# yynil/RWKV_LM_EXT

Measured on AMD Instinct MI355X. Metric: WKV6 fwd+bwd tokens/sec/GPU (B=8,T=4096,C=2048) + %HBM roofline, higher is better.
Workload: dtype bf16

## Files before the change

### rwkv_lm_ext_amd/csrc/wkv6_chunk_bwd12k.hip

```cpp
#include <type_traits>
#include "wkv6_chunk.h"

namespace wkv6 {

namespace {

using namespace chunk;

enum { R_RH = 0, R_RL, R_GY, R_R, R_K, NR_ARR };
enum { K_KH = 0, K_KL, K_V, NK_ARR };
constexpr int FRS = 72 * 4;
constexpr int ROFF_FR = NR_ARR * ARR;
constexpr int ROFF_LW = ROFF_FR + BLK * FRS;
constexpr int ROFF_E8 = ROFF_LW + BLK * FRS;
constexpr int ROFF_COEF = ROFF_E8 + 256;
constexpr int ROFF_VG = ROFF_COEF + 128;
constexpr int RBLK_BYTES = ROFF_VG + 128;
constexpr int KOFF_E16 = NK_ARR * ARR;
constexpr int KOFF_E16M8 = KOFF_E16 + 256;
constexpr int KBLK_BYTES = KOFF_E16M8 + 256;
constexpr int STG = 32, SBLK = STG / BLK;
constexpr int RBUF_BYTES = SBLK * RBLK_BYTES;
constexpr int KBUF_BYTES = SBLK * KBLK_BYTES;
constexpr int KRING = 3;
constexpr int KP_OFF = 2 * RBUF_BYTES;
constexpr int CKT = CKPT_TOK;
constexpr int XT_OFF = KP_OFF + KRING * KBUF_BYTES;
constexpr int XS_OFF = XT_OFF + 4 * 1024;
constexpr int XFLAG_OFF = 128;
constexpr int GRS = 144;
constexpr int GOP_OFF = XS_OFF + 2 * 1024;
constexpr int TAG_DA = 0, TAG_SC = 4, TAG_GA = 8, TAG_GB = 12, TAG_GC = 16, TAG_GD = 20, N_TAGS = 24;
constexpr int BWD12K_LDS = GOP_OFF + 2 * HEAD * GRS;
static_assert(BWD12K_LDS <= 160 * 1024, "LDS budget");

#define WKV6_DPP_ACC4(x, ctrl) asm("s_nop 1\n\t" \
    "v_add_f32_dpp %0, %0, %0 " ctrl " row_mask:0xf bank_mask:0xf\n\t" "v_add_f32_dpp %1, %1, %1 " ctrl " row_mask:0xf bank_mask:0xf\n\t" \
    "v_add_f32_dpp %2, %2, %2 " ctrl " row_mask:0xf bank_mask:0xf\n\t" "v_add_f32_dpp %3, %3, %3 " ctrl " row_mask:0xf bank_mask:0xf" \
    : "+v"(x[0]), "+v"(x[1]), "+v"(x[2]), "+v"(x[3]))

enum : unsigned {
    BWD_W_RAW = 1u << 0,
    BWD_SPLIT = 1u << 1,
    BWD_AFF = 1u << 2,
    BWD_CLK = 1u << 3,
    BWD_CHAIN = 1u << 4,
    BWD_VARLEN = 1u << 5,
};
constexpr unsigned bit(bool on, unsigned b) { return on ? b : 0u; }
struct BwdChain {
    int b, ntok;
    int ko, ro;
    bool chained_in;
    bool nx_chain;
    unsigned nx_bh;
    int nx_b, nx_ntok;
    bool nx_rev, nx_use_u;
    const float* nx_ckpt;
};
struct BwdCarry {
    uint2 pr[2], pk[2], pw[2];
    float4 pe[2];
    uint2 ck_[2];
    float cfr[2][4], clw[2][4], cc8[4];
    uint2 cvp[2];
    f4v CK[4];
};
template <unsigned MODE, int GEN = 0, int ROLE = 0>
__device__ __forceinline__ void chunk_bwd12k_body(const ScanArgs& a, const unsigned slot, BwdCarry& cy, const unsigned sslot = 0, const BwdChain& ch = BwdChain{})
{
    constexpr bool W_RAW = (MODE & BWD_W_RAW) != 0;
    constexpr bool SPLIT = (MODE & BWD_SPLIT) != 0;
    constexpr bool AFF = (MODE & BWD_AFF) != 0;
    constexpr bool CLK = (MODE & BWD_CLK) != 0;
    constexpr bool CHAIN = (MODE & BWD_CHAIN) != 0;
    constexpr bool VARLEN = (MODE & BWD_VARLEN) != 0;
    [[maybe_unused]] const bool chained_in = CHAIN && ch.chained_in, nx_chain = CHAIN && ch.nx_chain;
    [[maybe_unused]] const int ko = CHAIN ? ch.ko : 0, ro = CHAIN ? ch.ro : 0;
    extern __shared__ __attribute__((aligned(16))) char smem[];
    int tid_ = threadIdx.x;
    if constexpr (CHAIN) asm volatile("" : "+v"(tid_));
    const int tid = tid_, lane = tid & 63;
    const SplitForms spf = split_forms(lane);
    const int hwid = __builtin_amdgcn_readfirstlane(tid >> 6);
    const int part = SPLIT ? (int)(slot & 1) : 0;
    const int bh = SPLIT ? (int)(slot >> 1) : (int)slot;
    const int wid = SPLIT ? (hwid < 4 ? hwid + 4 * part : hwid + 4) : hwid;
    const bool rowrole = ROLE ? ROLE == 1 : wid < 4, producer = ROLE ? ROLE == 3 : wid >= 8;
    const int wv = wid & 3;
    const int pb = wid & 1, half = (wid >> 1) & 1;
    const int b = CHAIN ? ch.b : (a.order ? a.order[bh / a.H] : bh / a.H), h = bh % a.H;
    const long base = VARLEN ? (long)a.tok_off[b] * a.C + (long)h * HEAD : (long)b * a.T * a.C + (long)h * HEAD;
    const bf16_t* const gr_ = reinterpret_cast<const bf16_t*>(a.r) + base;
    const bf16_t* const gk_ = reinterpret_cast<const bf16_t*>(a.k) + base;
    const bf16_t* const gv_ = reinterpret_cast<const bf16_t*>(a.v) + base;
    const bf16_t* const ggy = reinterpret_cast<const bf16_t*>(a.gy) + base;
    bf16_t* const ogr = reinterpret_cast<bf16_t*>(a.gr) + base;
    bf16_t* const ogk = reinterpret_cast<bf16_t*>(a.gk) + base;
    bf16_t* const ogv = reinterpret_cast<bf16_t*>(a.gv) + base;
    bf16_t* const ogw = reinterpret_cast<bf16_t*>(a.gw) + base;
    int ntok = a.T;
    if constexpr (CHAIN) ntok = ch.ntok;
    else if (a.lens) ntok = min(max(a.lens[b], 0), a.T);
    const TokAddr<AFF> tok(a, b, ntok);
    const int C_ = a.C;
    const unsigned nbytes = ntok > 0 ? (unsigned)(ntok - 1) * a.C * 2u + 128u : 0u;
    const rsrc_t rs_gr = make_rsrc(ogr, nbytes), rs_gk = make_rsrc(ogk, nbytes), rs_gv = make_rsrc(ogv, nbytes), rs_gw = make_rsrc(ogw, nbytes);
    const long sbase = (GEN && a.side_compact) ? (long)sslot * a.T * HEAD : base;
    const unsigned sstr = (GEN && a.side_compact) ? (unsigned)HEAD : (unsigned)a.C;
    const unsigned nbytes4 = ntok > 0 ? (unsigned)(ntok - 1) * sstr * 4u + 256u : 0u;
    const rsrc_t rs_side[4] = {make_rsrc(GEN && a.g_f32[0] ? a.g_f32[0] + sbase : nullptr, GEN && a.g_f32[0] ? nbytes4 : 0u),
                               make_rsrc(GEN && a.g_f32[1] ? a.g_f32[1] + sbase : nullptr, GEN && a.g_f32[1] ? nbytes4 : 0u),
                               make_rsrc(GEN && a.g_f32[2] ? a.g_f32[2] + sbase : nullptr, GEN && a.g_f32[2] ? nbytes4 : 0u),
                               make_rsrc(GEN && a.g_f32[3] ? a.g_f32[3] + sbase : nullptr, GEN && a.g_f32[3] ? nbytes4 : 0u)};
    const int lp_side = tok.lane(lane & 15, 16 * wv + 4 * (lane >> 4), (int)sstr);
    const int lp_put = tok.lane((((lane >> 4) & 1) ? 0 : BLK) + (lane & 15), 16 * wv + 8 * (lane >> 5), C_);
    auto fetch_old = [&](int which, const rsrc_t& rs, int pu, unsigned bit, float (&old)[4]) {
        if constexpr (GEN == 2) {
            const unsigned idx = tok.off(pu, lane & 15, 16 * wv + 4 * (lane >> 4), (int)sstr, bit, lp_side);
            const float4 t = buf_load16f(rs_side[which], idx * 4u);
            old[0] = t.x; old[1] = t.y; old[2] = t.z; old[3] = t.w;
        }
    };
#ifdef WKV6_STAMP
    unsigned long long stamp_acc[6] = {0, 0, 0, 0, 0, 0}, ts0 = 0, ts1 = 0, ts2 = 0, ts3 = 0, ts4 = 0, ts5 = 0;
    unsigned long long tp0 = 0, tp1 = 0;
    unsigned long long poll_acc[8] = {0, 0, 0, 0, 0, 0, 0, 0};
#define WKV6_ACCP(idx, t1, t0) do { stamp_acc[5] += (t1) - (t0); poll_acc[(idx) >> 2] += (t1) - (t0); } while (0)
#else
#define WKV6_ACCP(idx, t1, t0) do { } while (0)
#endif
    const int x_ = lane & 15, g_ = lane >> 4;
    typedef unsigned v2u_t __attribute__((ext_vector_type(2)));
    typedef unsigned v4u_t __attribute__((ext_vector_type(4)));
    typedef volatile v4u_t __attribute__((address_space(3))) lds_vv4u;
    [[maybe_unused]] uint2 held_st[4] = {};
    auto put = [&](int which, const rsrc_t& rs, int stg, int blk, unsigned bit, uint2 v) {
        if constexpr (GEN == 1) return;
        if (blk == SBLK - 1) { held_st[which] = v; return; }
        const auto sx = __builtin_amdgcn_permlane16_swap(held_st[which].x, v.x, false, false);
        const auto sy = __builtin_amdgcn_permlane16_swap(held_st[which].y, v.y, false, false);
        buf_store16(rs, tok.off(stg * STG, ((g_ & 1) ? 0 : BLK) + x_, 16 * wv + 8 * (g_ >> 1), C_, bit, lp_put) * 2u,
                    make_uint4(sx[0], sy[0], sx[1], sy[1]));
    };
    auto emit = [&](int which, int stg, int blk, unsigned bit, float (&o)[4], const float (&old)[4]) -> uint2 {
        if constexpr (GEN == 1) {
            const unsigned idx = tok.off(stg * STG + blk * BLK, x_, 16 * wv + 4 * g_, (int)sstr, bit, lp_side);
            buf_store16f(rs_side[which], idx * 4u, o);
            return make_uint2(0u, 0u);
        }
        if constexpr (GEN == 2) {
#pragma unroll
            for (int q = 0; q < 4; ++q) o[q] += old[q];
        }
        return make_uint2(pack_bf2(o[0], o[1]), pack_bf2(o[2], o[3]));
    };

#ifdef WKV6_DEBUGBUF
    unsigned long long clk0 = 0, rtc0 = 0, clk1 = 0, rtc1 = 0;
    WKV6_CLK(clk0, rtc0);
#endif
    if constexpr (CLK) { if (hwid == 0) clock_stamp(a, slot, 0); }
    const int ngrp = (ntok + STG - 1) / STG;
    auto rpart = [&](int stg, int blk) { return smem + ((stg + ro) & 1) * RBUF_BYTES + blk * RBLK_BYTES; };
    auto kpart = [&](int stg, int blk) { return smem + KP_OFF + (int)((unsigned)(stg + ko) % (unsigned)KRING) * KBUF_BYTES + blk * KBLK_BYTES; };
    [[maybe_unused]] auto rpart_nx = [&](int e, int blk) { return smem + ((ro + 1 + e) & 1) * RBUF_BYTES + blk * RBLK_BYTES; };
    [[maybe_unused]] auto kpart_nx = [&](int e, int blk) { return smem + KP_OFF + (int)((unsigned)(ko + 2 * KRING - 1 - e) % (unsigned)KRING) * KBUF_BYTES + blk * KBLK_BYTES; };

    const int c8i = lane & 7, tq = lane >> 3;
    const int ch0 = 32 * half + 4 * c8i;
    float uu[4] = {0.f, 0.f, 0.f, 0.f};
    if (a.use_u) io4<bf16_t>::load(reinterpret_cast<const bf16_t*>(a.u) + h * HEAD + ch0, uu);

    uint2 (&pr)[2] = cy.pr, (&pk)[2] = cy.pk, (&pw)[2] = cy.pw;
    float4 (&pe)[2] = cy.pe;
    uint2 (&ck_)[2] = cy.ck_;
    uint2 pv[2], pg[2], cv_[2];
    float (&cfr)[2][4] = cy.cfr, (&clw)[2][4] = cy.clw, (&cc8)[4] = cy.cc8;
    if (!chained_in) { cc8[0] = 0.f; cc8[1] = 0.f; cc8[2] = 0.f; cc8[3] = 0.f; }
    const rsrc_t rs_r = make_rsrc(gr_, nbytes), rs_k = make_rsrc(gk_, nbytes), rs_v = make_rsrc(gv_, nbytes), rs_g = make_rsrc(ggy, nbytes);
    const rsrc_t rs_w = W_RAW ? make_rsrc(reinterpret_cast<const bf16_t*>(a.w) + base, nbytes)
                              : make_rsrc(reinterpret_cast<const float*>(a.w) + base, ntok > 0 ? (unsigned)(ntok - 1) * a.C * 4u + 256u : 0u);
    struct RowIn {
        rsrc_t r, k, v, g, w;
        TokAddr<AFF> tok;
    };
    const RowIn cur{rs_r, rs_k, rs_v, rs_g, rs_w, tok};
    [[maybe_unused]] auto row_in_of = [&](int b_, int h_, int ntok_, bool rev_) {
        const long base_ = (long)b_ * a.T * a.C + (long)h_ * HEAD;
        const unsigned nb_ = ntok_ > 0 ? (unsigned)(ntok_ - 1) * a.C * 2u + 128u : 0u;
        return RowIn{make_rsrc(reinterpret_cast<const bf16_t*>(a.r) + base_, nb_), make_rsrc(reinterpret_cast<const bf16_t*>(a.k) + base_, nb_),
                     make_rsrc(reinterpret_cast<const bf16_t*>(a.v) + base_, nb_), make_rsrc(reinterpret_cast<const bf16_t*>(a.gy) + base_, nb_),
                     W_RAW ? make_rsrc(reinterpret_cast<const bf16_t*>(a.w) + base_, nb_)
                           : make_rsrc(reinterpret_cast<const float*>(a.w) + base_, ntok_ > 0 ? (unsigned)(ntok_ - 1) * a.C * 4u + 256u : 0u),
                     TokAddr<AFF>(ntok_, rev_)};
    };
    const int lp_in[2] = {tok.lane(pb * BLK + 2 * tq, ch0, C_), tok.lane(pb * BLK + 2 * tq + 1, ch0, C_)};
    auto load_r = [&](const RowIn& in, const int (&lp)[2], int stg) {
#pragma unroll
        for (int tt = 0; tt < 2; ++tt) {
            pr[tt] = buf_load8(in.r, in.tok.off(stg * STG, pb * BLK + 2 * tq + tt, ch0, C_, REV_R, lp[tt]) * 2u);
            if constexpr (SPLIT) pg[tt] = buf_load8(in.g, in.tok.off(stg * STG, pb * BLK + 2 * tq + tt, ch0, C_, REV_Y, lp[tt]) * 2u);
        }
    };
    auto load_kw = [&](const RowIn& in, const int (&lp)[2], int stg) {
#pragma unroll
        for (int tt = 0; tt < 2; ++tt) {
            const int pl = pb * BLK + 2 * tq + tt;
            const unsigned ik = in.tok.off(stg * STG, pl, ch0, C_, REV_K, lp[tt]), iw = in.tok.off(stg * STG, pl, ch0, C_, REV_W, lp[tt]);
            pk[tt] = buf_load8(in.k, ik * 2u);
            if constexpr (SPLIT) pv[tt] = buf_load8(in.v, in.tok.off(stg * STG, pl, ch0, C_, REV_V, lp[tt]) * 2u);
            if constexpr (W_RAW) pw[tt] = buf_load8(in.w, iw * 2u);
            else pe[tt] = buf_load16f(in.w, iw * 4u);
        }
    };
    auto prep = [&](auto HASR, auto HASK, char* const rb, char* const kb, int sk, int ntok_k, const float (&uu)[4],
                    const RowIn& rq, const int (&rq_lp)[2], int next_r, int next_k) {
        float r[2][4], ko[2][4], k[2][4], cs[2][4], lwn[2][4], coef[2] = {0.f, 0.f};
        if constexpr (HASR) {
#pragma unroll
            for (int tt = 0; tt < 2; ++tt) {
                r[tt][0] = bf_lo(pr[tt].x); r[tt][1] = bf_hi(pr[tt].x); r[tt][2] = bf_lo(pr[tt].y); r[tt][3] = bf_hi(pr[tt].y);
                ko[tt][0] = bf_lo(ck_[tt].x); ko[tt][1] = bf_hi(ck_[tt].x); ko[tt][2] = bf_lo(ck_[tt].y); ko[tt][3] = bf_hi(ck_[tt].y);
                float part = 0.f;
#pragma unroll
                for (int c = 0; c < 4; ++c) part = fmaf(r[tt][c] * uu[c], ko[tt][c], part);
                part += dpp_mov<DPP_XOR1>(part);
                part += dpp_mov<DPP_XOR2>(part);
                part += dpp_mov<DPP_SHL4>(part);
                coef[tt] = part;
                const int tok = 2 * tq + tt;
                char* const rowz = rb + tok * RSB + ((ch0 * 2) ^ ((tok & 8) << 1));
                *reinterpret_cast<uint2*>(rowz + R_R * ARR) = pr[tt];
                *reinterpret_cast<uint2*>(rowz + R_K * ARR) = ck_[tt];
                *reinterpret_cast<float4*>(rb + ROFF_LW + tok * FRS + ch0 * 4) = make_float4(clw[tt][0], clw[tt][1], clw[tt][2], clw[tt][3]);
                if constexpr (SPLIT) {
                    *reinterpret_cast<uint2*>(rb + tok * RSB + ch0 * 2 + R_GY * ARR) = pg[tt];
                    typedef __bf16 bf2 __attribute__((ext_vector_type(2)));
                    float pvg = __builtin_amdgcn_fdot2_f32_bf16(__builtin_bit_cast(bf2, pg[tt].x), __builtin_bit_cast(bf2, cv_[tt].x), 0.f, false);
                    pvg = __builtin_amdgcn_fdot2_f32_bf16(__builtin_bit_cast(bf2, pg[tt].y), __builtin_bit_cast(bf2, cv_[tt].y), pvg, false);
                    pvg += dpp_mov<DPP_XOR1>(pvg);
                    pvg += dpp_mov<DPP_XOR2>(pvg);
                    pvg += dpp_mov<DPP_SHL4>(pvg);
                    if (c8i == 0) *reinterpret_cast<float*>(rb + ROFF_VG + (half * 16 + tok) * 4) = pvg;
                }
            }
        }
        if constexpr (HASR) load_r(rq, rq_lp, next_r);
        if constexpr (HASK) {
#pragma unroll
            for (int tt = 0; tt < 2; ++tt) {
                const bool valid = sk * STG + pb * BLK + 2 * tq + tt < ntok_k;
                k[tt][0] = bf_lo(pk[tt].x); k[tt][1] = bf_hi(pk[tt].x); k[tt][2] = bf_lo(pk[tt].y); k[tt][3] = bf_hi(pk[tt].y);
                ck_[tt] = pk[tt];
                if constexpr (SPLIT) {
                    *reinterpret_cast<uint2*>(kb + (2 * tq + tt) * RSB + ch0 * 2 + K_V * ARR) = pv[tt];
                    cv_[tt] = pv[tt];
                }
                float lw[4];
                if constexpr (W_RAW) {
                    lw[0] = -exp2_fast(LOG2E * bf_lo(pw[tt].x)); lw[1] = -exp2_fast(LOG2E * bf_hi(pw[tt].x));
                    lw[2] = -exp2_fast(LOG2E * bf_lo(pw[tt].y)); lw[3] = -exp2_fast(LOG2E * bf_hi(pw[tt].y));
                } else {
                    lw[0] = pe[tt].x; lw[1] = pe[tt].y; lw[2] = pe[tt].z; lw[3] = pe[tt].w;
                }
#pragma unroll
                for (int c = 0; c < 4; ++c) {
                    const float l = valid ? fmaxf(lw[c] * LOG2E, LW_MIN2) : 0.f;
                    cs[tt][c] = tt ? cs[tt - 1][c] + l : l;
                    lwn[tt][c] = valid ? lw[c] : 0.f;
                }
            }
            if (__builtin_amdgcn_ballot_w64(lwn[0][0] < LW_MIN || lwn[0][1] < LW_MIN || lwn[0][2] < LW_MIN || lwn[0][3] < LW_MIN ||
                                            lwn[1][0] < LW_MIN || lwn[1][1] < LW_MIN || lwn[1][2] < LW_MIN || lwn[1][3] < LW_MIN)) {
#pragma unroll
                for (int tt = 0; tt < 2; ++tt)
#pragma unroll
                    for (int c = 0; c < 4; ++c) lwn[tt][c] *= exp2_fast(LOG2E * fminf(lwn[tt][c] - LW_MIN, 0.f));
            }
            load_kw(rq, rq_lp, next_k);
        } else {
#pragma unroll
            for (int tt = 0; tt < 2; ++tt)
#pragma unroll
                for (int c = 0; c < 4; ++c) { k[tt][c] = 0.f; cs[tt][c] = 0.f; lwn[tt][c] = 0.f; }
        }
        float pre[4], c8[4], c16[4];
#pragma unroll
        for (int c = 0; c < 4; ++c) {
            float tot = cs[1][c], a_, b_;
            const float t = dpp_mov<DPP_ROR8>(tot);
            float pfx = (tq & 1) ? t : 0.f;
            tot += t;
            rows16(tot, a_, b_);
            pfx += (tq & 2) ? a_ : 0.f;
            tot = a_ + b_;
            halves32(tot, a_, b_);
            pfx += (tq & 4) ? a_ : 0.f;
            pre[c] = pfx;
            c8[c] = a_;
            c16[c] = a_ + b_;
        }
        if constexpr (HASR) {
#pragma unroll
            for (int tt = 0; tt < 2; ++tt) {
                float rh[4], fr[4];
#pragma unroll
                for (int c = 0; c < 4; ++c) {
                    fr[c] = exp2_fast(cfr[tt][c]);
                    rh[c] = r[tt][c] * fr[c];
                }
                const int tok = 2 * tq + tt;
                char* const row = rb + tok * RSB + ch0 * 2;
                uint2 hi, lo;
                split4(rh, hi, lo, spf.form<MS_BWD_PROD>());
                *reinterpret_cast<uint2*>(row + R_RH * ARR) = hi; *reinterpret_cast<uint2*>(row + R_RL * ARR) = lo;
                *reinterpret_cast<float4*>(rb + ROFF_FR + tok * FRS + ch0 * 4) = make_float4(fr[0], fr[1], fr[2], fr[3]);
            }
        }
#pragma unroll
        for (int tt = 0; tt < 2; ++tt) {
            float kh[4];
#pragma unroll
            for (int c = 0; c < 4; ++c) {
                const float cex = tt ? pre[c] + cs[tt - 1][c] : pre[c];
                const float cin = pre[c] + cs[tt][c];
                cfr[tt][c] = cex - c8[c];
                clw[tt][c] = lwn[tt][c];
                kh[c] = k[tt][c] * exp2_fast(c8[c] - cin);
            }
            if constexpr (HASK) {
                char* const row = kb + (2 * tq + tt) * RSB + ch0 * 2;
                uint2 hi, lo;
                split4(kh, hi, lo, spf.form<MS_BWD_PROD>());
                *reinterpret_cast<uint2*>(row + K_KH * ARR) = hi; *reinterpret_cast<uint2*>(row + K_KL * ARR) = lo;
            }
        }
        if constexpr (HASR) {
            if (c8i == 0) {
                *reinterpret_cast<float*>(rb + ROFF_COEF + (half * 16 + 2 * tq) * 4) = coef[0];
                *reinterpret_cast<float*>(rb + ROFF_COEF + (half * 16 + 2 * tq + 1) * 4) = coef[1];
            }
        }
        if (tq == 0) {
            if constexpr (HASR)
                *reinterpret_cast<float4*>(rb + ROFF_E8 + ch0 * 4) =
                    make_float4(exp2_fast(cc8[0]), exp2_fast(cc8[1]), exp2_fast(cc8[2]), exp2_fast(cc8[3]));
            if constexpr (HASK) {
                *reinterpret_cast<float4*>(kb + KOFF_E16 + ch0 * 4) =
                    make_float4(exp2_fast(c16[0]), exp2_fast(c16[1]), exp2_fast(c16[2]), exp2_fast(c16[3]));
                *reinterpret_cast<float4*>(kb + KOFF_E16M8 + ch0 * 4) =
                    make_float4(exp2_fast(c16[0] - c8[0]), exp2_fast(c16[1] - c8[1]), exp2_fast(c16[2] - c8[2]), exp2_fast(c16[3] - c8[3]));
            }
        }
#pragma unroll
        for (int c = 0; c < 4; ++c) cc8[c] = c8[c];
    };

    const int x = lane & 15, g = lane >> 4;
    int troff = (4 * g + (x >> 2)) * RSB + 8 * (x & 3);
    int trow = (4 * g + (x >> 2)) * RSB + 16 * (x & 3);
    auto cat2 = [](s4v a_, s4v b_) { return __builtin_bit_cast(b8v, __builtin_shufflevector(a_, b_, 0, 1, 2, 3, 4, 5, 6, 7)); };
    typedef volatile int __attribute__((address_space(3))) lds_vint;
    auto xflag_at = [&](int idx) { return (lds_vint*)(smem + (idx >> 3) * RSB + XFLAG_OFF + (idx & 7) * 4); };
    if (tid < N_TAGS) *xflag_at(tid) = 0;
    unsigned tag_wv = (unsigned)(unsigned long)(lds_vint*)(smem + XFLAG_OFF + 4 * wv);
    unsigned tag_tb = (unsigned)(unsigned long)(lds_vint*)(smem + XFLAG_OFF + 8 * (wv & 1));
    asm volatile("" : "+v"(tag_wv), "+v"(tag_tb));
    auto tag_off = [](int idx0) { return (idx0 >> 3) * RSB + (idx0 & 7) * 4; };
    auto publish_at = [&](unsigned base, int idx0, int extra, int tagv) {
        if (lane == 0) *(lds_vint*)(unsigned long)(base + (unsigned)(tag_off(idx0) + extra)) = tagv;
    };
    auto publish = [&](int idx0, int tagv) { publish_at(tag_wv, idx0, 0, tagv); };
#ifdef WKV6_DEBUG
    auto spin_fail = [&](int idx, int tag, unsigned seen) {
        if (a.aux && lane == 0) {
            unsigned* const d = reinterpret_cast<unsigned*>(a.aux);
            d[0] = 0xdeadbeefu; d[1] = slot; d[2] = (unsigned)((wid << 8) | idx); d[3] = (unsigned)tag; d[4] = seen;
        }
        __builtin_trap();
    };
#define WKV6_SPIN_GUARD(idx, tag, seen) if (++spins > (1u << 22)) spin_fail(idx, tag, seen)
#else
#define WKV6_SPIN_GUARD(idx, tag, seen) do { } while (0)
#endif
    const int lane_tag4 = (lane & 3) * 4, lane_tag2 = (lane & 1) * 4;
    auto tags_differ = [&](unsigned f, int tag) { return __builtin_amdgcn_ballot_w64(f != (unsigned)tag) != 0; };
    auto await_n = [&](int idx, int tag, int lane_off) {
        [[maybe_unused]] unsigned spins = 0;
        WKV6_T(tp0);
        for (;;) {
            const unsigned f = (unsigned)*(lds_vint*)((unsigned char __attribute__((address_space(3)))*)xflag_at(idx) + lane_off);
            if (!tags_differ(f, tag)) break;
            WKV6_SPIN_GUARD(idx, tag, f);
            __builtin_amdgcn_s_sleep(1);
        }
        WKV6_T(tp1); WKV6_ACCP(idx, tp1, tp0);
    };
    auto await2 = [&](int idx, int tag) { await_n(idx, tag, lane_tag2); };
    auto await4 = [&](int idx, int tag) { await_n(idx, tag, lane_tag4); };
    auto peek4 = [&](int idx) -> unsigned {
        return (unsigned)*(lds_vint*)((unsigned char __attribute__((address_space(3)))*)xflag_at(idx) + lane_tag4);
    };
    auto settle4 = [&](int idx, int tag, const unsigned f) { if (tags_differ(f, tag)) await4(idx, tag); };
    auto tile_store = [&](int off, uint2 hi, uint2 lo) {
        *(lds_vv4u*)(smem + off + lane * 16) = v4u_t{hi.x, hi.y, lo.x, lo.y};
    };
    auto tile_load = [&](int off) {
        const v4u_t f = *(lds_vv4u*)(smem + off + lane * 16);
        return make_uint4(f.x, f.y, f.z, f.w);
    };
    constexpr std::true_type yes_c{};
    constexpr std::false_type no_c{};
    [[maybe_unused]] const int nxn = CHAIN ? (ch.nx_ntok + STG - 1) / STG : 0;
    if (producer) {
        if (!chained_in && ngrp > 0) {
            load_kw(cur, lp_in, ngrp - 1);
            load_r(cur, lp_in, ngrp - 1);
            prep(no_c, yes_c, rpart(0, pb), kpart(ngrp - 1, pb), ngrp - 1, ntok, uu, cur, lp_in, -1, ngrp - 2);
            if (ngrp > 1) prep(yes_c, yes_c, rpart(ngrp - 1, pb), kpart(ngrp - 2, pb), ngrp - 2, ntok, uu, cur, lp_in, ngrp - 2, ngrp - 3);
            else prep(yes_c, no_c, rpart(0, pb), kpart(0, pb), -1, ntok, uu, cur, lp_in, -1, -1);
        }
        __syncthreads();
        for (int grp = ngrp - 1; grp >= 2; --grp) {
            WKV6_T(ts0);
#ifdef WKV6_STAMP
            asm volatile("" :: "v"(pr[0].x), "v"(pk[0].x), "v"(pr[1].x), "v"(pk[1].x));
#endif
            WKV6_T(ts1);
            WKV6_T(ts2);
            prep(yes_c, yes_c, rpart(grp - 1, pb), kpart(grp - 2, pb), grp - 2, ntok, uu, cur, lp_in, grp - 2, grp - 3);
            WKV6_T(ts3);
            __syncthreads();
            WKV6_T(ts4);
            WKV6_ACC(0, ts1, ts0); WKV6_ACC(1, ts2, ts1); WKV6_ACC(2, ts3, ts2); WKV6_ACC(3, ts4, ts3);
        }
        bool chained_out = false;
        if constexpr (CHAIN) {
            if (nx_chain) {
                const int nxh = (int)(ch.nx_bh % (unsigned)a.H);
                const RowIn nx = row_in_of(ch.nx_b, nxh, ch.nx_ntok, ch.nx_rev);
                const int lp_nx[2] = {nx.tok.lane(pb * BLK + 2 * tq, ch0, C_), nx.tok.lane(pb * BLK + 2 * tq + 1, ch0, C_)};
                float uu_nx[4] = {0.f, 0.f, 0.f, 0.f};
                if (ch.nx_use_u) io4<bf16_t>::load(reinterpret_cast<const bf16_t*>(a.u) + nxh * HEAD + ch0, uu_nx);
                load_kw(nx, lp_nx, nxn - 1);
                prep(yes_c, yes_c, rpart(0, pb), kpart_nx(0, pb), nxn - 1, ch.nx_ntok, uu, nx, lp_nx, nxn - 1, nxn - 2);
                __syncthreads();
                prep(yes_c, yes_c, rpart_nx(0, pb), kpart_nx(1, pb), nxn - 2, ch.nx_ntok, uu_nx, nx, lp_nx, nxn - 2, nxn - 3);
                __syncthreads();
                chained_out = true;
            }
        }
        if (!chained_out) {
            if (ngrp >= 2) {
                prep(yes_c, no_c, rpart(0, pb), kpart(0, pb), -1, ntok, uu, cur, lp_in, -1, -1);
                __syncthreads();
            }
            if (ngrp >= 1) __syncthreads();
        }
    } else
    if (rowrole) {
        float ue[4] = {0.f, 0.f, 0.f, 0.f};
        if (a.use_u) io4<bf16_t>::load(reinterpret_cast<const bf16_t*>(a.u) + h * HEAD + 16 * wv + 4 * g, ue);
        f4v ST[SBLK][4], GI[4];
#pragma unroll
        for (int t = 0; t < 4; ++t) GI[t] = f4v{0.f, 0.f, 0.f, 0.f};
        float Rc[4] = {0.f, 0.f, 0.f, 0.f}, gu_acc[4] = {0.f, 0.f, 0.f, 0.f};
        if (a.rc_in) io4<float>::load(a.rc_in + (long)b * a.C + h * HEAD + 16 * wv + 4 * g, Rc);
        const unsigned nslots = VARLEN ? ((unsigned)ntok + CKT - 1) / CKT : ((unsigned)a.T + CKT - 1) / CKT;
        const int segs = a.ckpt_segs > 1 ? a.ckpt_segs : 1;
        const long ck_slot0 = VARLEN ? (long)h * a.ck_stride + a.ck_off[b] : ((long)((b / segs) * a.H + h) * segs + b % segs) * nslots;
        const rsrc_t rs_ck = make_rsrc(a.ckpt + ck_slot0 * (HEAD * HEAD), nslots * 16384u);
        f4v (&CK)[4] = cy.CK;
        auto request_ckpt = [&](int stg) {
            const unsigned off = (unsigned)(stg >> 1) * 16384u + (unsigned)wv * 4096u + (unsigned)lane * 16u;
#pragma unroll
            for (int jt = 0; jt < 4; ++jt) {
                const float4 t = buf_load16f(rs_ck, off + jt * 1024u);
                CK[jt] = f4v{t.x, t.y, t.z, t.w};
            }
        };
        auto advance = [&](const char* kb, const f4v (&Sin)[4], f4v (&Sout)[4]) {
            const s4v khf = tr_read(kb + K_KH * ARR + troff + 32 * wv);
            const s4v klf = tr_read(kb + K_KL * ARR + troff + 32 * wv);
            const float e16 = *reinterpret_cast<const float*>(kb + KOFF_E16 + (16 * wv + x) * 4);
            const float e16m8 = *reinterpret_cast<const float*>(kb + KOFF_E16M8 + (16 * wv + x) * 4);
#pragma unroll
            for (int jt = 0; jt < 4; ++jt) {
                const s4v vf = tr_read(kb + K_V * ARR + trow + tile_tr(jt));
                f4v o = {0.f, 0.f, 0.f, 0.f};
                o = mfma32(cat2(vf, vf), cat2(khf, klf), o);
#pragma unroll
                for (int q = 0; q < 4; ++q) Sout[jt][q] = fmaf(e16, Sin[jt][q], e16m8 * o[q]);
            }
        };
        if constexpr (CHAIN) { if (!chained_in && ngrp > 0) request_ckpt(ngrp - 1); }
#pragma unroll
        for (int q = 0; q < 4; ++q) asm volatile("" : "+v"(ue[q]), "+v"(Rc[q]));
        if constexpr (!CHAIN) { if (ngrp > 0) request_ckpt(ngrp - 1); }
        {
            unsigned none_bytes = 0u;
            if constexpr (CHAIN) { asm volatile("" : "+s"(none_bytes)); none_bytes = __builtin_amdgcn_readfirstlane(none_bytes); }
            const rsrc_t rs_none = make_rsrc(static_cast<bf16_t*>(nullptr), none_bytes);
#pragma unroll
            for (int i = 0; i < (GEN == 1 ? 4 : 3); ++i)
                buf_store16(rs_none, 16u * i, make_uint4(__float_as_uint(ue[0]), __float_as_uint(ue[1]), __float_as_uint(ue[2]), __float_as_uint(ue[3])));
        }

        __syncthreads();
        for (int grp = ngrp - 1; grp >= 0; --grp) {
            int tagv = grp + 1;
            asm volatile("" : "+v"(tagv));
            WKV6_T(ts0);
            f4v gvb[SBLK];
            auto take_gop = [&](int blk) {
                int base_ = GOP_OFF + (8 * g + (x >> 2)) * GRS + (16 * wv + 4 * (x & 3)) * 2;
                asm volatile("" : "+v"(base_));
                typedef short s8v __attribute__((ext_vector_type(8)));
                const char* const kb = kpart(grp, blk);
                f4v acc = {0.f, 0.f, 0.f, 0.f};
#pragma unroll
                for (int s = 0; s < 2; ++s) {
                    const char* const ph = smem + base_ + 32 * s * GRS;
                    const s8v h8 = __builtin_shufflevector(tr_read(ph), tr_read(ph + 4 * GRS), 0, 1, 2, 3, 4, 5, 6, 7);
                    const s8v l8 = __builtin_shufflevector(tr_read(ph + HEAD * GRS), tr_read(ph + HEAD * GRS + 4 * GRS), 0, 1, 2, 3, 4, 5, 6, 7);
                    const b8v vr = ld_b8(kb + K_V * ARR + x * RSB + (32 * s + 8 * g) * 2);
                    acc = mfma32(__builtin_bit_cast(b8v, h8), vr, acc);
                    acc = mfma32(__builtin_bit_cast(b8v, l8), vr, acc);
                }
                return acc;
            };
            if constexpr (!SPLIT) {
                if (grp == ngrp - 1) await4(TAG_GA, grp + 1);
                gvb[1] = take_gop(1);
                publish(TAG_GB, tagv);
            }
            float old_gr[SBLK][4] = {}, old_gk[SBLK][4] = {}, old_gw[SBLK][4] = {};
#pragma unroll
            for (int blk = SBLK - 1; blk >= 0; --blk) fetch_old(0, rs_gr, grp * STG + blk * BLK, REV_R, old_gr[blk]);
            if (wv >= 2) {
                const int tb = wv - 2;
                const char* const rb = rpart(grp, tb);
                const char* const kb = kpart(grp, tb);
                f4v dA_ab = {0.f, 0.f, 0.f, 0.f}, dA_ba = {0.f, 0.f, 0.f, 0.f};
#pragma unroll
                for (int s = 0; s < 2; ++s) {
                    const int off = x * RSB + (32 * s + 8 * g) * 2;
                    const b8v gy_ = ld_b8(rb + R_GY * ARR + off), vr = ld_b8(kb + K_V * ARR + off);
                    dA_ab = mfma32(gy_, vr, dA_ab);
                    dA_ba = mfma32(vr, gy_, dA_ba);
                }
                float dab[4], dba[4];
#pragma unroll
                for (int q = 0; q < 4; ++q) {
                    const int o = 4 * g + q;
                    dab[q] = x < o ? dA_ab[q] : 0.f;
                    dba[q] = o < x ? dA_ba[q] : 0.f;
                }
                uint2 th, tl;
                split4(dab, th, tl, spf.form<MS_BWD_TILE>());
                tile_store(XT_OFF + (2 * tb) * 1024, th, tl);
                publish_at(tag_tb, TAG_DA, 0, tagv);
                split4(dba, th, tl, spf.form<MS_BWD_TILE>());
                tile_store(XT_OFF + (2 * tb + 1) * 1024, th, tl);
                publish_at(tag_tb, TAG_DA, 4, tagv);
            } else if constexpr (!SPLIT) {
                const char* const rb = rpart(grp, wv);
                const char* const kb = kpart(grp, wv);
                f4v sc = {0.f, 0.f, 0.f, 0.f};
#pragma unroll
                for (int s = 0; s < 2; ++s) {
                    const int off = x * RSB + (32 * s + 8 * g) * 2;
                    const b8v rh = ld_b8(rb + R_RH * ARR + off), rl = ld_b8(rb + R_RL * ARR + off);
                    const b8v kh = ld_b8(kb + K_KH * ARR + off), kl = ld_b8(kb + K_KL * ARR + off);
                    sc = mfma32(rh, kh, sc);
                    sc = mfma32(rh, kl, sc);
                    sc = mfma32(rl, kh, sc);
                }
                const float4 cfa = *reinterpret_cast<const float4*>(rb + ROFF_COEF + 16 * g);
                const float4 cfb = *reinterpret_cast<const float4*>(rb + ROFF_COEF + 64 + 16 * g);
                const float cf[4] = {cfa.x + cfb.x, cfa.y + cfb.y, cfa.z + cfb.z, cfa.w + cfb.w};
                float scm[4];
#pragma unroll
                for (int q = 0; q < 4; ++q) {
                    const int o = 4 * g + q;
                    scm[q] = x < o ? sc[q] : (x == o ? cf[q] : 0.f);
                }
                uint2 th, tl;
                split4(scm, th, tl, spf.form<MS_BWD_TILE>());
                tile_store(XS_OFF + wv * 1024, th, tl);
                publish(TAG_SC, tagv);
            }
#pragma unroll
            for (int jt = 0; jt < 4; ++jt) ST[0][jt] = CK[jt];
            WKV6_T(ts1);
            if (grp & 1) {
                advance(kpart(grp - 1, 0), ST[0], ST[0]);
                advance(kpart(grp - 1, 1), ST[0], ST[0]);
            }
            [[maybe_unused]] unsigned pk_gc = 0;
#pragma unroll
            for (int blk = 0; blk < SBLK - 1; ++blk) advance(kpart(grp, blk), ST[blk], ST[blk + 1]);
            const unsigned pk_da = peek4(TAG_DA);
            WKV6_T(ts2);
            f4v ackp[SBLK];
            float at[SBLK][4], vgs[SBLK];
            uint2 held_gr[SBLK];
#pragma unroll
            for (int blk = SBLK - 1; blk >= 0; --blk) {
                const char* const rb = rpart(grp, blk);
                const char* const kb = kpart(grp, blk);
                b8v gyr[2];
#pragma unroll
                for (int s = 0; s < 2; ++s) gyr[s] = ld_b8(rb + R_GY * ARR + x * RSB + (32 * s + 8 * g) * 2);
                const float vg = *reinterpret_cast<const float*>(rb + ROFF_VG + x * 4) + *reinterpret_cast<const float*>(rb + ROFF_VG + 64 + x * 4);
                vgs[blk] = vg;
                if (blk == SBLK - 1) settle4(TAG_DA, grp + 1, pk_da);
                if constexpr (!SPLIT) { if (blk == 0) pk_gc = peek4(TAG_GC); }
                const uint4 fab = tile_load(XT_OFF + (2 * blk) * 1024), fba = tile_load(XT_OFF + (2 * blk + 1) * 1024);
                const s4v dab_hi = __builtin_bit_cast(s4v, make_uint2(fab.x, fab.y)), dab_lo = __builtin_bit_cast(s4v, make_uint2(fab.z, fab.w));
                const s4v dba_hi = __builtin_bit_cast(s4v, make_uint2(fba.x, fba.y)), dba_lo = __builtin_bit_cast(s4v, make_uint2(fba.z, fba.w));
                const s4v rhf_w = tr_read(rb + R_RH * ARR + troff + 32 * wv);
                const s4v rlf_w = tr_read(rb + R_RL * ARR + troff + 32 * wv);
                const s4v khf = tr_read(kb + K_KH * ARR + troff + 32 * wv);
                const s4v klf = tr_read(kb + K_KL * ARR + troff + 32 * wv);
                const float4 e8o = *reinterpret_cast<const float4*>(rb + ROFF_E8 + (16 * wv + 4 * g) * 4);
                f4v accs = {0.f, 0.f, 0.f, 0.f};
#pragma unroll
                for (int s = 0; s < 2; ++s) {
                    float t0[4], t1[4];
                    b8v hi, lo;
#pragma unroll
                    for (int q = 0; q < 4; ++q) { t0[q] = ST[blk][2 * s][q]; t1[q] = ST[blk][2 * s + 1][q]; }
                    split8(t0, t1, hi, lo, spf.form<MS_BWD_ROW>());
                    accs = mfma32(hi, gyr[s], accs);
                    accs = mfma32(lo, gyr[s], accs);
                }
                f4v accr16 = {0.f, 0.f, 0.f, 0.f};
                accr16 = mfma16(khf, dba_hi, accr16);
                accr16 = mfma16(khf, dba_lo, accr16);
                accr16 = mfma16(klf, dba_hi, accr16);
                const f4v accr = {fmaf(e8o.x, accs[0], accr16[0]), fmaf(e8o.y, accs[1], accr16[1]),
                                  fmaf(e8o.z, accs[2], accr16[2]), fmaf(e8o.w, accs[3], accr16[3])};
                f4v ak = {0.f, 0.f, 0.f, 0.f};
                ak = mfma16(rhf_w, dab_hi, ak);
                ak = mfma16(rhf_w, dab_lo, ak);
                ak = mfma16(rlf_w, dab_hi, ak);
                ackp[blk] = ak;
                {
                    const int ch = 16 * wv + 4 * g;
                    const float4 fr4 = *reinterpret_cast<const float4*>(rb + ROFF_FR + x * FRS + ch * 4);
                    const uint2 rr = *reinterpret_cast<const uint2*>(rb + R_R * ARR + x * RSB + ((ch * 2) ^ ((x & 8) << 1)));
                    const uint2 kk = *reinterpret_cast<const uint2*>(rb + R_K * ARR + x * RSB + ((ch * 2) ^ ((x & 8) << 1)));
                    const float frv[4] = {fr4.x, fr4.y, fr4.z, fr4.w};
                    const float rv[4] = {bf_lo(rr.x), bf_hi(rr.x), bf_lo(rr.y), bf_hi(rr.y)};
                    const float kv[4] = {bf_lo(kk.x), bf_hi(kk.x), bf_lo(kk.y), bf_hi(kk.y)};
                    float o_gr[4];
#pragma unroll
                    for (int q = 0; q < 4; ++q) {
                        const float dq = frv[q] * accr[q];
                        o_gr[q] = fmaf(vg * ue[q], kv[q], dq);
                        gu_acc[q] = fmaf(vg * rv[q], kv[q], gu_acc[q]);
                        at[blk][q] = rv[q] * dq;
                    }
                    held_gr[blk] = emit(0, grp, blk, REV_R, o_gr, old_gr[blk]);
                }
            }
            WKV6_T(ts3);
#pragma unroll
            for (int blk = SBLK - 1; blk >= 0; --blk) {
                fetch_old(1, rs_gk, grp * STG + blk * BLK, REV_K, old_gk[blk]);
                fetch_old(3, rs_gw, grp * STG + blk * BLK, REV_W, old_gw[blk]);
            }
            if (grp > 0 && !(grp & 1)) request_ckpt(grp - 1);
            if constexpr (CHAIN) {
                if (nx_chain && grp == 0) {
                    const rsrc_t rs_nx = make_rsrc(ch.nx_ckpt + ((long)ch.nx_b * a.H + (long)(ch.nx_bh % (unsigned)a.H)) * nslots * (HEAD * HEAD), nslots * 16384u);
                    const unsigned off = (unsigned)((nxn - 1) >> 1) * 16384u + (unsigned)wv * 4096u + (unsigned)lane * 16u;
#pragma unroll
                    for (int jt = 0; jt < 4; ++jt) {
                        const float4 t = buf_load16f(rs_nx, off + jt * 1024u);
                        CK[jt] = f4v{t.x, t.y, t.z, t.w};
                    }
                }
            }
            if constexpr (!SPLIT) {
                settle4(TAG_GC, grp + 1, pk_gc);
                gvb[0] = take_gop(0);
                publish(TAG_GD, tagv);
            }
#pragma unroll
            for (int blk = SBLK - 1; blk >= 0; --blk) put(0, rs_gr, grp, blk, REV_R, held_gr[blk]);
#pragma unroll
            for (int blk = SBLK - 1; blk >= 0; --blk) {
                const char* const rb = rpart(grp, blk);
                const char* const kb = kpart(grp, blk);
                f4v acck = {0.f, 0.f, 0.f, 0.f};
                [[maybe_unused]] f4v Oi[4];
                [[maybe_unused]] float e8x = 0.f, e16x = 0.f;
                if constexpr (SPLIT) {
                    e8x = *reinterpret_cast<const float*>(rb + ROFF_E8 + (16 * wv + x) * 4);
                    e16x = *reinterpret_cast<const float*>(kb + KOFF_E16 + (16 * wv + x) * 4);
                    const float e16m8x = *reinterpret_cast<const float*>(kb + KOFF_E16M8 + (16 * wv + x) * 4);
                    const s4v rhf_w = tr_read(rb + R_RH * ARR + troff + 32 * wv);
                    const s4v rlf_w = tr_read(rb + R_RL * ARR + troff + 32 * wv);
#pragma unroll
                    for (int jt = 0; jt < 4; ++jt) {
                        const s4v gyf = tr_read(rb + R_GY * ARR + trow + tile_tr(jt));
                        f4v o = {0.f, 0.f, 0.f, 0.f};
                        o = mfma32(cat2(gyf, gyf), cat2(rhf_w, rlf_w), o);
                        Oi[jt] = o;
                    }
#pragma unroll
                    for (int s = 0; s < 2; ++s) {
                        const b8v vr = ld_b8(kb + K_V * ARR + x * RSB + (32 * s + 8 * g) * 2);
                        float t0[4], t1[4];
                        b8v hi, lo;
#pragma unroll
                        for (int q = 0; q < 4; ++q) { t0[q] = GI[2 * s][q] * e16m8x; t1[q] = GI[2 * s + 1][q] * e16m8x; }
                        split8(t0, t1, hi, lo, spf.form<MS_BWD_ROW>());
                        acck = mfma32(hi, vr, acck);
                        acck = mfma32(lo, vr, acck);
                    }
                } else {
                    acck = gvb[blk];
                }
                acck += ackp[blk];
                {
                    const int ch = 16 * wv + 4 * g;
                    const float4 fn4 = *reinterpret_cast<const float4*>(x < 15 ? rb + ROFF_FR + (x + 1) * FRS + ch * 4 : kb + KOFF_E16M8 + ch * 4);
                    const float4 fk4 = make_float4(__builtin_amdgcn_rcpf(fn4.x), __builtin_amdgcn_rcpf(fn4.y), __builtin_amdgcn_rcpf(fn4.z),
                                                   __builtin_amdgcn_rcpf(fn4.w));
                    const float4 lw4 = *reinterpret_cast<const float4*>(rb + ROFF_LW + x * FRS + ch * 4);
                    const uint2 rr = *reinterpret_cast<const uint2*>(rb + R_R * ARR + x * RSB + ((ch * 2) ^ ((x & 8) << 1)));
                    const uint2 kk = *reinterpret_cast<const uint2*>(rb + R_K * ARR + x * RSB + ((ch * 2) ^ ((x & 8) << 1)));
                    const float fkv[4] = {fk4.x, fk4.y, fk4.z, fk4.w}, lwv[4] = {lw4.x, lw4.y, lw4.z, lw4.w};
                    const float rv[4] = {bf_lo(rr.x), bf_hi(rr.x), bf_lo(rr.y), bf_hi(rr.y)};
                    const float kv[4] = {bf_lo(kk.x), bf_hi(kk.x), bf_lo(kk.y), bf_hi(kk.y)};
                    const float vg = vgs[blk];
                    float o_gk[4], o_gw[4], bt[4], dl[4], sfx[4];
#pragma unroll
                    for (int q = 0; q < 4; ++q) {
                        const float dk = fkv[q] * acck[q];
                        o_gk[q] = fmaf(vg * ue[q], rv[q], dk);
                        bt[q] = kv[q] * dk;
                        dl[q] = at[blk][q] - bt[q];
                        sfx[q] = dl[q];
                    }
                    WKV6_DPP_ACC4(sfx, "row_shl:1");
                    WKV6_DPP_ACC4(sfx, "row_shl:2");
                    WKV6_DPP_ACC4(sfx, "row_shl:4");
                    WKV6_DPP_ACC4(sfx, "row_shl:8");
#pragma unroll
                    for (int q = 0; q < 4; ++q) {
                        const float total = dpp_mov<DPP_BCAST0>(sfx[q]);
                        o_gw[q] = (Rc[q] + (sfx[q] - dl[q]) - bt[q]) * lwv[q];
                        Rc[q] += total;
                    }
                    put(1, rs_gk, grp, blk, REV_K, emit(1, grp, blk, REV_K, o_gk, old_gk[blk]));
                    put(3, rs_gw, grp, blk, REV_W, emit(3, grp, blk, REV_W, o_gw, old_gw[blk]));
                }
                if constexpr (SPLIT) {
#pragma unroll
                    for (int jt = 0; jt < 4; ++jt)
#pragma unroll
                        for (int q = 0; q < 4; ++q) GI[jt][q] = fmaf(e16x, GI[jt][q], e8x * Oi[jt][q]);
                }
            }
            WKV6_T(ts4);
            __syncthreads();
            WKV6_T(ts5);
            WKV6_ACC(0, ts1, ts0); WKV6_ACC(1, ts2, ts1); WKV6_ACC(2, ts3, ts2); WKV6_ACC(3, ts4, ts3); WKV6_ACC(4, ts5, ts4);
        }
        if (a.gu) {
            float s4[4];
#pragma unroll
            for (int q = 0; q < 4; ++q) s4[q] = row_sum16(gu_acc[q]);
            const long o = (long)b * a.C + h * HEAD + 16 * wv + 4 * g;
            if (x == 0) {
                if (a.part_f32) io4<float>::store(reinterpret_cast<float*>(a.gu) + o, s4);
                else io4<bf16_t>::store(reinterpret_cast<bf16_t*>(a.gu) + o, s4);
            }
        }
    } else {
        f4v GJ[4];
#pragma unroll
        for (int t = 0; t < 4; ++t) {
            float t4[4] = {0.f, 0.f, 0.f, 0.f};
            if (a.g_in)
                io4<float>::load(a.g_in + ((long)b * a.H + h) * HEAD * HEAD + (long)(16 * wv + x) * HEAD + tile_ch(t) + 8 * g, t4);
            GJ[t] = f4v{t4[0], t4[1], t4[2], t4[3]};
        }
#pragma unroll
        for (int t = 0; t < 4; ++t) asm volatile("" : "+v"(GJ[t]));
        const int tl = lane >> 4, cl = lane & 15;
        uint2 cv[SBLK], cg[SBLK];
        uint2 (&cvp)[SBLK] = cy.cvp;
        const int lp_vg = tok.lane(4 * wv + tl, 4 * cl, C_);
        auto load_v = [&](const RowIn& in, int lp, int stg) {
#pragma unroll
            for (int blk = 0; blk < SBLK; ++blk) {
                cv[blk] = buf_load8(in.v, in.tok.off(stg * STG + blk * BLK, 4 * wv + tl, 4 * cl, C_, REV_V, lp) * 2u);
            }
        };
        auto load_gy = [&](const RowIn& in, int lp, int stg) {
#pragma unroll
            for (int blk = 0; blk < SBLK; ++blk) {
                cg[blk] = buf_load8(in.g, in.tok.off(stg * STG + blk * BLK, 4 * wv + tl, 4 * cl, C_, REV_Y, lp) * 2u);
            }
        };
        auto copy_v = [&](char* const k0) {
#pragma unroll
            for (int blk = 0; blk < SBLK; ++blk) {
                *reinterpret_cast<uint2*>(k0 + blk * KBLK_BYTES + K_V * ARR + (4 * wv + tl) * RSB + 8 * cl) = cv[blk];
                cvp[blk] = cv[blk];
            }
        };
        auto copy_gy = [&](char* const r0) {
#pragma unroll
            for (int blk = 0; blk < SBLK; ++blk) {
                char* const rb = r0 + blk * RBLK_BYTES;
                const int tok = 4 * wv + tl;
                *reinterpret_cast<uint2*>(rb + R_GY * ARR + tok * RSB + 8 * cl) = cg[blk];
                typedef __bf16 bf2 __attribute__((ext_vector_type(2)));
                float vg = __builtin_amdgcn_fdot2_f32_bf16(__builtin_bit_cast(bf2, cg[blk].x), __builtin_bit_cast(bf2, cvp[blk].x), 0.f, false);
                vg = __builtin_amdgcn_fdot2_f32_bf16(__builtin_bit_cast(bf2, cg[blk].y), __builtin_bit_cast(bf2, cvp[blk].y), vg, false);
                vg += dpp_mov<DPP_XOR1>(vg);
                vg += dpp_mov<DPP_XOR2>(vg);
                vg += dpp_mov<DPP_SHL4>(vg);
                if ((cl & 7) == 0) *reinterpret_cast<float*>(rb + ROFF_VG + ((cl >> 3) * 16 + tok) * 4) = vg;
            }
        };
        [[maybe_unused]] RowIn nx = cur;
        [[maybe_unused]] int lp_vg_nx = lp_vg;
        if constexpr (CHAIN) {
            if (nx_chain) {
                nx = row_in_of(ch.nx_b, (int)(ch.nx_bh % (unsigned)a.H), ch.nx_ntok, ch.nx_rev);
                lp_vg_nx = nx.tok.lane(4 * wv + tl, 4 * cl, C_);
            }
        }
        auto scale_split = [&](const char* kb, b8v (&h)[2], b8v (&l)[2]) {
#pragma unroll
            for (int s = 0; s < 2; ++s) {
                float t0[4], t1[4];
                const float4 m0 = *reinterpret_cast<const float4*>(kb + KOFF_E16M8 + (32 * s + 8 * g) * 4);
                const float4 m1 = *reinterpret_cast<const float4*>(kb + KOFF_E16M8 + (32 * s + 8 * g + 4) * 4);
                t0[0] = GJ[2 * s][0] * m0.x; t0[1] = GJ[2 * s][1] * m0.y; t0[2] = GJ[2 * s][2] * m0.z; t0[3] = GJ[2 * s][3] * m0.w;
                t1[0] = GJ[2 * s + 1][0] * m1.x; t1[1] = GJ[2 * s + 1][1] * m1.y;
                t1[2] = GJ[2 * s + 1][2] * m1.z; t1[3] = GJ[2 * s + 1][3] * m1.w;
                split8(t0, t1, h[s], l[s], spf.form<MS_BWD_COL>());
            }
        };
        auto gop_write = [&](const b8v (&h)[2], const b8v (&l)[2]) {
#pragma unroll
            for (int s = 0; s < 2; ++s) {
                char* const dst = smem + GOP_OFF + (16 * wv + x) * GRS + (32 * s + 8 * g) * 2;
                *(lds_vv4u*)dst = __builtin_bit_cast(v4u_t, h[s]);
                *(lds_vv4u*)(dst + HEAD * GRS) = __builtin_bit_cast(v4u_t, l[s]);
            }
        };
        [[maybe_unused]] b8v nh[2] = {}, nl[2] = {};
        if (!SPLIT && !chained_in && ngrp > 0) {
            load_v(cur, lp_vg, ngrp - 1);
            load_gy(cur, lp_vg, ngrp - 1);
            copy_v(kpart(ngrp - 1, 0));
            copy_gy(rpart(ngrp - 1, 0));
            if (ngrp > 1) {
                load_v(cur, lp_vg, ngrp - 2);
                copy_v(kpart(ngrp - 2, 0));
            }
        }
        __syncthreads();
        if constexpr (!SPLIT) { if (ngrp > 0) scale_split(kpart(ngrp - 1, SBLK - 1), nh, nl); }
        for (int grp = ngrp - 1; grp >= 0; --grp) {
            int tagv = grp + 1;
            for (int i_ = 0; i_ < wv; ++i_) __builtin_amdgcn_s_sleep(2);
            asm volatile("" : "+v"(tagv));
            WKV6_T(ts0);

            s4v gyT_w[SBLK], sc_hi[SBLK], sc_lo[SBLK];
            f4v accp[SBLK];
            b8v gh[SBLK][2], gl[SBLK][2];
            [[maybe_unused]] f4v Og[SBLK][4];
            if constexpr (!SPLIT)
#pragma unroll
            for (int blk = SBLK - 1; blk >= 0; --blk) {
                const char* const rb = rpart(grp, blk);
                const char* const kb = kpart(grp, blk);
                if (blk == SBLK - 1) {
#pragma unroll
                    for (int s = 0; s < 2; ++s) { gh[blk][s] = nh[s]; gl[blk][s] = nl[s]; }
                    if (grp == ngrp - 1) {
                        gop_write(gh[blk], gl[blk]);
                        publish(TAG_GA, tagv);
                    }
                    if constexpr (CHAIN) {
                        const bool g_nx = nx_chain && grp == 0, v_nx = nx_chain && grp <= 1;
                        load_gy(g_nx ? nx : cur, g_nx ? lp_vg_nx : lp_vg, g_nx ? nxn - 1 : grp - 1);
                        load_v(v_nx ? nx : cur, v_nx ? lp_vg_nx : lp_vg, v_nx ? (grp == 1 ? nxn - 1 : nxn - 2) : grp - 2);
                    } else {
                        if (grp > 0) load_gy(cur, lp_vg, grp - 1);
                        if (grp > 1) load_v(cur, lp_vg, grp - 2);
                    }
                } else {
                    scale_split(kb, gh[blk], gl[blk]);
                    await4(TAG_GB, grp + 1);
                    gop_write(gh[blk], gl[blk]);
                    publish(TAG_GC, tagv);
                }
                const s4v gyT = tr_read(rb + R_GY * ARR + troff + 32 * wv);
#pragma unroll
                for (int it = 0; it < 4; ++it) {
                    const s4v rhf = tr_read(rb + R_RH * ARR + trow + tile_tr(it));
                    const s4v rlf = tr_read(rb + R_RL * ARR + trow + tile_tr(it));
                    f4v o = {0.f, 0.f, 0.f, 0.f};
                    o = mfma32(cat2(rhf, rlf), cat2(gyT, gyT), o);
                    const float4 d16 = *reinterpret_cast<const float4*>(kb + KOFF_E16 + (tile_ch(it) + 8 * g) * 4);
                    const float4 d8 = *reinterpret_cast<const float4*>(rb + ROFF_E8 + (tile_ch(it) + 8 * g) * 4);
                    GJ[it][0] = fmaf(d16.x, GJ[it][0], d8.x * o[0]);
                    GJ[it][1] = fmaf(d16.y, GJ[it][1], d8.y * o[1]);
                    GJ[it][2] = fmaf(d16.z, GJ[it][2], d8.z * o[2]);
// ... 383 lines not shown
```

Baseline: 57.55 million.

## Stage gr/gk/gw outputs through LDS and flush them with coalesced 16-byte stores

In the plain (non-split, non-chained, GEN 0) backward path, row-role waves no longer issue scattered 8-byte global stores for gr, gk and gw. They stash those results into the stage's R/K/LW LDS slots. Producer waves then flush each finished stage with 16-byte buffer stores in a token-major layout, one stage behind, and the producer prologue is shifted by one group to make room. This targets uncoalesced store traffic and store issue on the compute waves, at the cost of extra LDS writes and reads, reuse of buffer regions, and a more complex prologue and epilogue that depend on synchronization ordering.

```diff
diff --git a/rwkv_lm_ext_amd/csrc/wkv6_chunk_bwd12k.hip b/rwkv_lm_ext_amd/csrc/wkv6_chunk_bwd12k.hip
--- a/rwkv_lm_ext_amd/csrc/wkv6_chunk_bwd12k.hip
+++ b/rwkv_lm_ext_amd/csrc/wkv6_chunk_bwd12k.hip
@@ -75,6 +75,7 @@
     constexpr bool CLK = (MODE & BWD_CLK) != 0;
     constexpr bool CHAIN = (MODE & BWD_CHAIN) != 0;
     constexpr bool VARLEN = (MODE & BWD_VARLEN) != 0;
+    constexpr bool STAGED = GEN == 0 && !SPLIT && !CHAIN;
     [[maybe_unused]] const bool chained_in = CHAIN && ch.chained_in, nx_chain = CHAIN && ch.nx_chain;
     [[maybe_unused]] const int ko = CHAIN ? ch.ko : 0, ro = CHAIN ? ch.ro : 0;
     extern __shared__ __attribute__((aligned(16))) char smem[];
@@ -114,7 +115,9 @@
                                make_rsrc(GEN && a.g_f32[2] ? a.g_f32[2] + sbase : nullptr, GEN && a.g_f32[2] ? nbytes4 : 0u),
                                make_rsrc(GEN && a.g_f32[3] ? a.g_f32[3] + sbase : nullptr, GEN && a.g_f32[3] ? nbytes4 : 0u)};
     const int lp_side = tok.lane(lane & 15, 16 * wv + 4 * (lane >> 4), (int)sstr);
-    const int lp_put = tok.lane((((lane >> 4) & 1) ? 0 : BLK) + (lane & 15), 16 * wv + 8 * (lane >> 5), C_);
+    int lp_put_ = tok.lane((((lane >> 4) & 1) ? 0 : BLK) + (lane & 15), 16 * wv + 8 * (lane >> 5), C_);
+    if constexpr (STAGED && AFF) asm volatile("" : "+v"(lp_put_));
+    const int lp_put = lp_put_;
     auto fetch_old = [&](int which, const rsrc_t& rs, int pu, unsigned bit, float (&old)[4]) {
         if constexpr (GEN == 2) {
             const unsigned idx = tok.off(pu, lane & 15, 16 * wv + 4 * (lane >> 4), (int)sstr, bit, lp_side);
@@ -167,6 +170,26 @@
     [[maybe_unused]] auto rpart_nx = [&](int e, int blk) { return smem + ((ro + 1 + e) & 1) * RBUF_BYTES + blk * RBLK_BYTES; };
     [[maybe_unused]] auto kpart_nx = [&](int e, int blk) { return smem + KP_OFF + (int)((unsigned)(ko + 2 * KRING - 1 - e) % (unsigned)KRING) * KBUF_BYTES + blk * KBLK_BYTES; };
 
+    [[maybe_unused]] auto stash = [&](int stg, int blk, uint2 gr4, uint2 gk4, uint2 gw4) {
+        char* const rb = rpart(stg, blk);
+        char* const rowz = rb + x_ * RSB + (((16 * wv + 4 * g_) * 2) ^ ((x_ & 8) << 1));
+        *reinterpret_cast<uint2*>(rowz + R_R * ARR) = gr4;
+        *reinterpret_cast<uint2*>(rowz + R_K * ARR) = gk4;
+        *reinterpret_cast<uint2*>(rb + ROFF_LW + x_ * FRS + (16 * wv + 4 * g_) * 4) = gw4;
+    };
+    const int ft = lane >> 2, fc = 32 * half + 8 * (lane & 3);
+    [[maybe_unused]] const int lp_fl = tok.lane(pb * BLK + ft, fc, C_);
+    [[maybe_unused]] auto flush = [&](int stg) {
+        const char* const rb = rpart(stg, pb);
+        const char* const rowz = rb + ft * RSB + ((fc * 2) ^ ((ft & 8) << 1));
+        const uint4 vr = *reinterpret_cast<const uint4*>(rowz + R_R * ARR), vk = *reinterpret_cast<const uint4*>(rowz + R_K * ARR);
+        const char* const lwz = rb + ROFF_LW + ft * FRS + fc * 4;
+        const uint2 w0 = *reinterpret_cast<const uint2*>(lwz), w1 = *reinterpret_cast<const uint2*>(lwz + 16);
+        buf_store16(rs_gr, tok.off(stg * STG, pb * BLK + ft, fc, C_, REV_R, lp_fl) * 2u, vr);
+        buf_store16(rs_gk, tok.off(stg * STG, pb * BLK + ft, fc, C_, REV_K, lp_fl) * 2u, vk);
+        buf_store16(rs_gw, tok.off(stg * STG, pb * BLK + ft, fc, C_, REV_W, lp_fl) * 2u, make_uint4(w0.x, w0.y, w1.x, w1.y));
+    };
+
     const int c8i = lane & 7, tq = lane >> 3;
     const int ch0 = 32 * half + 4 * c8i;
     float uu[4] = {0.f, 0.f, 0.f, 0.f};
@@ -422,8 +445,17 @@
             else prep(yes_c, no_c, rpart(0, pb), kpart(0, pb), -1, ntok, uu, cur, lp_in, -1, -1);
         }
         __syncthreads();
-        for (int grp = ngrp - 1; grp >= 2; --grp) {
+        int grp_top = ngrp - 1;
+        if constexpr (STAGED) {
+            if (grp_top >= 2) {
+                prep(yes_c, yes_c, rpart(grp_top - 1, pb), kpart(grp_top - 2, pb), grp_top - 2, ntok, uu, cur, lp_in, grp_top - 2, grp_top - 3);
+                __syncthreads();
+                --grp_top;
+            }
+        }
+        for (int grp = grp_top; grp >= 2; --grp) {
             WKV6_T(ts0);
+            if constexpr (STAGED) flush(grp + 1);
 #ifdef WKV6_STAMP
             asm volatile("" :: "v"(pr[0].x), "v"(pk[0].x), "v"(pr[1].x), "v"(pk[1].x));
 #endif
@@ -453,10 +485,15 @@
         }
         if (!chained_out) {
             if (ngrp >= 2) {
+                if constexpr (STAGED) { if (ngrp >= 3) flush(2); }
                 prep(yes_c, no_c, rpart(0, pb), kpart(0, pb), -1, ntok, uu, cur, lp_in, -1, -1);
                 __syncthreads();
-            }
-            if (ngrp >= 1) __syncthreads();
+                if constexpr (STAGED) flush(1);
+            }
+            if (ngrp >= 1) {
+                __syncthreads();
+                if constexpr (STAGED) flush(0);
+            }
         }
     } else
     if (rowrole) {
@@ -498,6 +535,7 @@
 #pragma unroll
         for (int q = 0; q < 4; ++q) asm volatile("" : "+v"(ue[q]), "+v"(Rc[q]));
         if constexpr (!CHAIN) { if (ngrp > 0) request_ckpt(ngrp - 1); }
+        if constexpr (!STAGED)
         {
             unsigned none_bytes = 0u;
             if constexpr (CHAIN) { asm volatile("" : "+s"(none_bytes)); none_bytes = __builtin_amdgcn_readfirstlane(none_bytes); }
@@ -689,8 +727,10 @@
                 gvb[0] = take_gop(0);
                 publish(TAG_GD, tagv);
             }
+            if constexpr (!STAGED)
 #pragma unroll
             for (int blk = SBLK - 1; blk >= 0; --blk) put(0, rs_gr, grp, blk, REV_R, held_gr[blk]);
+            [[maybe_unused]] uint2 held_gk[SBLK], held_gw[SBLK];
 #pragma unroll
             for (int blk = SBLK - 1; blk >= 0; --blk) {
                 const char* const rb = rpart(grp, blk);
@@ -757,8 +797,13 @@
                         o_gw[q] = (Rc[q] + (sfx[q] - dl[q]) - bt[q]) * lwv[q];
                         Rc[q] += total;
                     }
-                    put(1, rs_gk, grp, blk, REV_K, emit(1, grp, blk, REV_K, o_gk, old_gk[blk]));
-                    put(3, rs_gw, grp, blk, REV_W, emit(3, grp, blk, REV_W, o_gw, old_gw[blk]));
+                    if constexpr (STAGED) {
+                        held_gk[blk] = emit(1, grp, blk, REV_K, o_gk, old_gk[blk]);
+                        held_gw[blk] = emit(3, grp, blk, REV_W, o_gw, old_gw[blk]);
+                    } else {
+                        put(1, rs_gk, grp, blk, REV_K, emit(1, grp, blk, REV_K, o_gk, old_gk[blk]));
+                        put(3, rs_gw, grp, blk, REV_W, emit(3, grp, blk, REV_W, o_gw, old_gw[blk]));
+                    }
                 }
                 if constexpr (SPLIT) {
 #pragma unroll
@@ -767,6 +812,9 @@
                         for (int q = 0; q < 4; ++q) GI[jt][q] = fmaf(e16x, GI[jt][q], e8x * Oi[jt][q]);
                 }
             }
+            if constexpr (STAGED)
+#pragma unroll
+            for (int blk = SBLK - 1; blk >= 0; --blk) stash(grp, blk, held_gr[blk], held_gk[blk], held_gw[blk]);
             WKV6_T(ts4);
             __syncthreads();
             WKV6_T(ts5);
```

New measurement: 56.10 million. 0.975x the previous value.
